# apache/auron

Hardware: AMD Instinct MI355X
Metric: tpcds_suite_seconds (lower is better)
Workload: dtype decimal64/fp64

## Files before the change

### auron_amd/column.py

```python
from __future__ import annotations

from typing import Iterable, List, Optional, Sequence

import torch

from . import dtypes
from .dtypes import DataType


class Column:
    __slots__ = ("dtype", "data", "validity", "offsets")

    def __init__(
        self,
        dtype: DataType,
        data: torch.Tensor,
        validity: Optional[torch.Tensor] = None,
        offsets: Optional[torch.Tensor] = None,
    ):
        self.dtype = dtype
        self.data = data
        self.validity = validity
        self.offsets = offsets
        if dtype.uses_offsets:
# ... 77 lines not shown
                    limbs.append(((lo - (1 << 64)) if lo >= (1 << 63) else lo,
                                  iv >> 64))
                data = torch.tensor(limbs, dtype=torch.int64) if limbs else \
                    torch.empty((0, 2), dtype=torch.int64)
            else:
                data = torch.tensor(tvals, dtype=dtype.torch_dtype)
            col = Column(dtype, data, validity, None)
        assert len(col) == n
        return col.to(device)

    def to_pylist(self) -> list:
        c = self.to("cpu")
        valid = None if c.validity is None else c.validity.tolist()
        if self.dtype.is_string:
            raw = bytes(c.data.numpy().tobytes())
            offs = c.offsets.tolist()
            out = []
            for i in range(len(c)):
                if valid is not None and not valid[i]:
                    out.append(None)
                else:
                    out.append(raw[offs[i]:offs[i + 1]].decode("utf-8", errors="replace"))
            return out
        if self.dtype.is_list:
            offs = c.offsets.tolist()
            flat = c.data.tolist()
            out = []
            for i in range(len(c)):
                if valid is not None and not valid[i]:
                    out.append(None)
                else:
                    out.append(flat[offs[i]:offs[i + 1]])
            return out
        if self.dtype.code == dtypes.DECIMAL128:
            s = 10 ** self.dtype.scale
            lo = c.data[:, 0].tolist()
            hi = c.data[:, 1].tolist()
            m64 = (1 << 64) - 1
            vals = [((h << 64) | (l & m64)) / s for l, h in zip(lo, hi)]
            if valid is None:
                return vals
            return [v if ok else None for v, ok in zip(vals, valid)]
        vals = c.data.tolist()
        if self.dtype.code == dtypes.DECIMAL64:
            s = 10 ** self.dtype.scale
            vals = [v / s for v in vals]
        if valid is None:
            return vals
        return [v if ok else None for v, ok in zip(vals, valid)]

    def gather(self, indices: torch.Tensor,
               may_have_negative: bool = False) -> "Column":
        idx = indices.to(self.device)
        neg = None
        if may_have_negative and idx.numel():
            neg = idx < 0
            idx = idx.clamp(min=0)
            if not bool(neg.any()) if idx.device.type != "cuda" else False:
                neg = None
        validity = None
        if self.validity is not None:
            validity = self.validity[idx]
        if neg is not None:
            if validity is None:
                validity = torch.ones(idx.shape[0], dtype=torch.bool, device=self.device)
            validity = validity & ~neg
        if self.dtype.uses_offsets:
            off = self.offsets.to(torch.int64)
            starts = off[idx]
            lens = off[idx + 1] - starts
            if neg is not None:
                lens = torch.where(neg, torch.zeros_like(lens), lens)
            new_off = torch.zeros(idx.shape[0] + 1, dtype=torch.int64, device=self.device)
            torch.cumsum(lens, 0, out=new_off[1:])
            total = int(new_off[-1].item())
            if total == 0:
                out_el = torch.empty(0, dtype=self.data.dtype, device=self.device)
            elif self.device.type == "cuda" and self.data.dtype == torch.uint8:
                from . import native

                out_el = torch.empty(total, dtype=torch.uint8, device=self.device)
                rc = native.lib().au_bytes_gather(
                    self.data.data_ptr(), starts.contiguous().data_ptr(),
                    new_off.data_ptr(), out_el.data_ptr(), idx.shape[0],
                    native.stream_ptr(self.device))
                native.check(rc, "au_bytes_gather")
            else:
                pos = torch.arange(total, dtype=torch.int64, device=self.device)
                row = torch.repeat_interleave(lens)
                el_idx = pos - new_off[:-1][row] + starts[row]
                out_el = self.data[el_idx]
            return Column(self.dtype, out_el, validity, new_off)
        data = self.data[idx]
        return Column(self.dtype, data, validity, None)

    def filter(self, mask: torch.Tensor) -> "Column":
        idx = torch.nonzero(mask, as_tuple=False).flatten()
        return self.gather(idx)

    def slice(self, start: int, length: int) -> "Column":
        idx = torch.arange(start, start + length, dtype=torch.int64, device=self.device)
        return self.gather(idx)

    @staticmethod
    def concat(cols: List["Column"]) -> "Column":
        assert cols
# ... 99 lines not shown
            t = torch.from_numpy(np_arr)
            if t.dtype != dt.torch_dtype:
                t = t.to(dt.torch_dtype)
            col = Column(dt, t, validity, None)
        return col.to(device)

    def to_arrow(self):
        import numpy as np
        import pyarrow as pa

        c = self.to("cpu")
        mask = None
        if c.validity is not None:
            mask = ~c.validity.numpy()
        if self.dtype.is_string:
            vals = c.to_pylist()
            return pa.array(vals, type=pa.string())
        if self.dtype.code == dtypes.DECIMAL64:
            from decimal import Decimal

            sc = self.dtype.scale
            vals = [None if (mask is not None and mask[i])
                    else Decimal(int(c.data[i].item())).scaleb(-sc)
                    for i in range(len(c))]
            p = max(self.dtype.precision, sc + 1, 1)
            return pa.array(vals, type=pa.decimal128(p, sc))
        if self.dtype.code == dtypes.DECIMAL128:
            from decimal import Context, Decimal

            wide = Context(prec=80)
            sc = self.dtype.scale
            lo = c.data[:, 0].numpy()
            hi = c.data[:, 1].numpy()
            vals = []
            for i in range(len(c)):
                if mask is not None and mask[i]:
                    vals.append(None)
                else:
                    v = (int(hi[i]) << 64) | (int(lo[i]) & ((1 << 64) - 1))
                    vals.append(Decimal(v).scaleb(-sc, context=wide))
            p = max(self.dtype.precision, sc + 1, 1)
            return pa.array(vals, type=pa.decimal128(min(p, 38), sc))
        np_arr = c.data.numpy()
        if self.dtype.code == dtypes.TIMESTAMP:
            return pa.array(np_arr, from_pandas=False, mask=mask).cast(
                pa.timestamp("us"))
        return pa.array(np_arr, from_pandas=False, mask=mask)

    def __repr__(self) -> str:
        return f"Column({self.dtype.name}, n={len(self)}, nulls={self.null_count}, dev={self.device})"



def compact_validity(v: Optional[torch.Tensor]) -> Optional[torch.Tensor]:
    if v is None or v.device.type == "cuda":
        return v
    return None if bool(v.all()) else v


def adjacent_equal(c: Column, nan_equal: bool = False) -> torch.Tensor:
    n = len(c)
    if n <= 1:
        return torch.zeros(0, dtype=torch.bool, device=c.device)
    a = c.gather(torch.arange(0, n - 1, dtype=torch.int64, device=c.device))
    b = c.gather(torch.arange(1, n, dtype=torch.int64, device=c.device))
    if c.dtype.is_string:
        from . import strings as S

        eq = S.compare(a, b, "==")
    else:
        eq = a.data == b.data
        if nan_equal and c.dtype.is_float:
            eq = eq | (torch.isnan(a.data) & torch.isnan(b.data))
    ones = torch.ones(n - 1, dtype=torch.bool, device=c.device)
    av = a.validity if a.validity is not None else ones
    bv = b.validity if b.validity is not None else ones
    return (eq & av & bv) | (~av & ~bv)


class RecordBatch:
    __slots__ = ("names", "columns", "_eval_memo")

    def __init__(self, names: List[str], columns: List[Column]):
        assert len(names) == len(columns)
        if columns:
            n = len(columns[0])
            for c in columns:
                assert len(c) == n, f"ragged batch: {[len(x) for x in columns]}"
        self.names = list(names)
        self.columns = list(columns)

    @property
    def num_rows(self) -> int:
        return len(self.columns[0]) if self.columns else 0

    @property
    def num_columns(self) -> int:
        return len(self.columns)

    @property
    def device(self) -> torch.device:
        return self.columns[0].device if self.columns else torch.device("cpu")

    def column(self, name: str) -> Column:
        return self.columns[self.names.index(name)]

    def to(self, device) -> "RecordBatch":
        return RecordBatch(self.names, [c.to(device) for c in self.columns])

    def gather(self, idx: torch.Tensor,
               may_have_negative: bool = False) -> "RecordBatch":
        if self.device.type == "cuda" and len(self.columns) > 1:
            fused = self._gather_fused(idx, may_have_negative)
            if fused is not None:
                return fused
        return RecordBatch(self.names,
                           [c.gather(idx, may_have_negative) for c in self.columns])

    def _gather_fused(self, idx: torch.Tensor, may_have_negative: bool):
        from . import native

        if not native.available():
            return None
        import numpy as np

        lib = native.lib()
        idx = idx.to(self.device).to(torch.int64).contiguous()
        n = int(idx.numel())
        out_cols: list = [None] * len(self.columns)
        descs = []
        keep = [idx]
        for ci, c in enumerate(self.columns):
            if c.dtype.uses_offsets:
                out_cols[ci] = c.gather(idx, may_have_negative)
                continue
            data = c.data if c.data.is_contiguous() else c.data.contiguous()
            keep.append(data)
            esize = data.element_size() * (2 if c.dtype.code == dtypes.DECIMAL128 else 1)
            shape = (n, 2) if c.dtype.code == dtypes.DECIMAL128 else (n,)
            dst = torch.empty(shape, dtype=data.dtype, device=self.device)
            want_valid = c.validity is not None or may_have_negative
            dv = torch.empty(n, dtype=torch.bool, device=self.device) \
                if want_valid else None
            sv = 0
            if c.validity is not None:
                v = c.validity if c.validity.is_contiguous() else c.validity.contiguous()
                keep.append(v)
                sv = v.data_ptr()
            descs.append((data.data_ptr(), sv, dst.data_ptr(),
                          dv.data_ptr() if dv is not None else 0, esize, 0))
            out_cols[ci] = Column(c.dtype, dst, dv)
        if descs and n:
            arr = np.array(descs, dtype=np.uint64).reshape(-1, 6)
            arr = np.ascontiguousarray(arr)
            for lo in range(0, len(descs), 24):
                sub = np.ascontiguousarray(arr[lo:lo + 24])
                rc = lib.au_multi_gather(idx.data_ptr(), n, sub.ctypes.data,
                                         sub.shape[0],
                                         native.stream_ptr(self.device))
                native.check(rc, "au_multi_gather")
        return RecordBatch(self.names, out_cols)

    def filter(self, mask: torch.Tensor) -> "RecordBatch":
        idx = torch.nonzero(mask, as_tuple=False).flatten()
        return self.gather(idx)

    def slice(self, start: int, length: int) -> "RecordBatch":
        return RecordBatch(self.names, [c.slice(start, length) for c in self.columns])

    def select(self, names: Iterable[str]) -> "RecordBatch":
        names = list(names)
        return RecordBatch(names, [self.column(n) for n in names])

    @staticmethod
    def concat(batches: List["RecordBatch"]) -> "RecordBatch":
        assert batches
        names = batches[0].names
        cols = [Column.concat([b.columns[i] for b in batches]) for i in range(len(names))]
        return RecordBatch(names, cols)

    @staticmethod
    def from_pydict(d: dict, types: dict, device="cpu") -> "RecordBatch":
        names = list(d.keys())
        cols = [Column.from_pylist(d[n], types[n], device) for n in names]
        return RecordBatch(names, cols)
# ... 31 lines not shown
```

### auron_amd/config.py

```python
from __future__ import annotations

import os
from dataclasses import dataclass
from typing import Any, Dict, Optional


@dataclass(frozen=True)
class ConfigOption:
    key: str
    default: Any
    typ: type
    doc: str = ""
    env: Optional[str] = None


_REGISTRY: Dict[str, ConfigOption] = {}


def _opt(key: str, default, typ, doc="", env=None) -> ConfigOption:
    o = ConfigOption(key, default, typ, doc, env)
    _REGISTRY[key] = o
    return o


# ... 64 lines not shown
                               env="AURON_SORT_EXTERNAL_WIDE_KEYS")
EXCHANGE_SAMPLE_ROWS = _opt("spark.auron.rangePartition.sampleRows", 4096, int,
                            "per-rank sample size for range-partition bounds")
SCAN_CACHE_BYTES = _opt("spark.auron.scan.cache.maxBytes", 0, int,
                        "per-query decoded-scan cache budget; 0 = auto "
                        "(15% of HBM on GPU, 4 GB on CPU)",
                        env="AURON_SCAN_CACHE_BYTES")
STREAM_BYTES = _opt("spark.auron.stream.minInputBytes", -1, int,
                    "estimated agg-input bytes above which operators "
                    "stream instead of materializing; -1 = auto (8% of "
                    "HBM on GPU, 1 GB on CPU), 0 = always stream",
                    env="AURON_STREAM_BYTES")
SCAN_HBM_CACHE = _opt("spark.auron.scan.hbmStagedCache.maxBytes", 0, int,
                      "staged raw-page bytes kept device-resident across "
                      "reads; 0 = auto (30% of HBM)",
                      env="AURON_SCAN_HBM_CACHE")
HBM_CACHE_RESERVE = _opt("spark.auron.scan.hbmStagedCache.reserveFraction",
                         0.25, float,
                         "free-HBM fraction the staged-bytes cache must "
                         "never consume (evicts itself under pressure)")
SCAN_DELTA_NATIVE = _opt("spark.auron.scan.deltaNative.enable", True, bool,
                         "decode DELTA_BINARY_PACKED pages and "
                         "DELTA_LENGTH_BYTE_ARRAY / DELTA_BYTE_ARRAY string "
                         "pages with the k_pq_delta_* kernels from a "
                         "host-built miniblock index, DELTA_BYTE_ARRAY "
                         "strings rebuilt by k_pq_dba_bytes (off: "
                         "DELTA_BINARY_PACKED is expanded to PLAIN by one "
                         "host job per page and DELTA_LENGTH_BYTE_ARRAY and "
                         "DELTA_BYTE_ARRAY columns take the pyarrow host "
                         "read)",
                         env="AURON_SCAN_DELTA_NATIVE")
SCAN_PREFETCH = _opt("spark.auron.scan.streamPrefetch", 2, int,
                     "files decoded ahead of the consumer on the "
                     "streaming scan path")
SCAN_IO_THREADS = _opt("spark.auron.scan.ioThreads", 8, int,
                       "host page-read/staging thread-pool size",
                       env="AURON_SCAN_IO_THREADS")
STREAM_PEEK_FACTOR = _opt("spark.auron.stream.peekBatches", 8, int,
                          "batch-size multiples buffered before the "
                          "chunked agg commits to streaming")
STREAM_JOIN_PROBE = _opt("spark.auron.stream.joinProbe.enable", True, bool,
                         "probe build-right joins batch-by-batch on the "
                         "streaming path (GPU only)",
                         env="AURON_STREAM_JOIN_PROBE")
JOIN_FUSED_PROBE = _opt("spark.auron.join.fusedProbe.enable", True, bool,
                        "probe hash joins with the fused kernels "
                        "(k_join_probe_count / k_join_probe_fill / "
                        "k_join_exists: probe hash computed in-kernel, one "
                        "chain walk, per-tile offsets, key descriptors passed "
                        "by value) for up to 8 key columns (off: murmur3 + "
                        "k_join_count + torch scan + k_join_fill, and "
                        "join_counts for semi/anti/existence joins)",
                        env="AURON_JOIN_FUSED_PROBE")
DECIMAL128_NATIVE_ARITH = _opt("spark.auron.decimal128.nativeArith.enable",
                               True, bool,
                               "run exact decimal128 + - * /, comparisons, "
                               "casts, abs and CheckOverflow on the "
                               "k_dec128_* kernels (off: the exact "
                               "host-integer reference path, also on GPU "
                               "batches)",
                               env="AURON_DECIMAL128_NATIVE_ARITH")
SPILL_DIR = _opt("spark.auron.spill.dir", "", str,
                 "directory for disk-tier spill files (empty = system tmp)",
                 env="AURON_SPILL_DIR")
MEM_BUDGET = _opt("spark.auron.memory.budgetBytes", 0, int,
                  "absolute memmgr budget override; 0 = memoryFraction "
                  "of device/host memory", env="AURON_MEM_BUDGET")


class AuronConf:
    def __init__(self, overrides: Optional[Dict[str, Any]] = None):
        self._values: Dict[str, Any] = {}
        if overrides:
            for k, v in overrides.items():
                self.set(k, v)

    def set(self, key: str, value) -> "AuronConf":
        if key not in _REGISTRY:
            raise KeyError(f"unknown config {key}; known: {sorted(_REGISTRY)}")
        self._values[key] = value
        return self

    def get(self, opt: ConfigOption):
        if opt.key in self._values:
            return self._values[opt.key]
        if opt.env and opt.env in os.environ:
            raw = os.environ[opt.env]
            if opt.typ is bool:
                return raw not in ("0", "false", "False")
            return opt.typ(raw)
        return opt.default

    @staticmethod
    def options() -> Dict[str, ConfigOption]:
        return dict(_REGISTRY)
```

### auron_amd/engine/executor.py

```python
from __future__ import annotations

import os
import time
from dataclasses import dataclass, field
from typing import Dict, List, Optional

import torch
import torch.distributed as dist

from .. import dtypes, ops
from ..column import Column, RecordBatch, adjacent_equal, compact_validity
from ..dtypes import DataType
from ..exchange import all_gather_batch, all_to_all
from ..exprs import AggFunc, Col
from ..plan import nodes as P
from ..config import AGG_STREAMING, BROADCAST_CACHE_BYTES, AuronConf
from .window import exec_window


@dataclass
class ExecContext:
    device: torch.device = torch.device("cpu")
    rank: int = 0
    world_size: int = 1
# ... 50 lines not shown
    return None if p is None else (p, 0)


def _decimal128_key_type(a, b):
    if dtypes.DECIMAL128 not in (a.code, b.code):
        return None
    if a.code == b.code and a.scale == b.scale:
        return None
    oa, ob = _decimal_key_operand(a), _decimal_key_operand(b)
    if oa is None or ob is None:
        return None
    (p1, s1), (p2, s2) = oa, ob
    s = max(s1, s2)
    digits = max(p1 - s1, p2 - s2)
    if s + digits > dtypes.MAX_DECIMAL_PRECISION:
        return None
    return dtypes.decimal128(s + digits, s)


def _normalize_join_keys(lkeys, rkeys):
    from ..exprs import _cast_col, _promote

    lo, ro = [], []
    for l, r in zip(lkeys, rkeys):
        common = _decimal128_key_type(l.dtype, r.dtype)
        if common is not None:
            l, r = _cast_col(l, common), _cast_col(r, common)
        elif (l.dtype.code == r.dtype.code == dtypes.DECIMAL128
              and l.dtype.scale != r.dtype.scale):
            l = _cast_col(l, dtypes.float64)
            r = _cast_col(r, dtypes.float64)
        elif l.dtype.code != r.dtype.code:
            l, r, _ = _promote(l, r)
        lo.append(l)
        ro.append(r)
    return lo, ro


class TaskCancelled(RuntimeError):
    """Raised inside execute() after Executor.cancel()."""


def _cast_for_range(c: Column) -> Column:
    if c.dtype.is_string:
        raise NotImplementedError("range partitioning on string keys")
    return c


def _concat(batches: List[RecordBatch]) -> RecordBatch:
    assert batches, "executor invariant violated: empty batch list"
    if len(batches) == 1:
        return batches[0]
    return RecordBatch.concat(batches)


def _empty_like(batch: RecordBatch) -> RecordBatch:
    idx = torch.empty(0, dtype=torch.int64, device=batch.device)
    return batch.gather(idx)



def _expr_sig(exprs) -> bytes:
    import hashlib

    from ..plan.serde import serialize_plan
    from ..plan import serde as _serde
    import msgpack as _mp

    return hashlib.sha1(_mp.packb([_serde._encode(e) for e in exprs],
                                  use_bin_type=True)).digest()


def _cacheable_build(plan) -> bool:
    if isinstance(plan, (P.MemoryScan, P.PyUdf, P.PyUdaf, P.Generate)):
        return False
    return all(_cacheable_build(c) for c in plan.children())


class Executor:
    def __init__(self, ctx: Optional[ExecContext] = None):
        self.ctx = ctx or ExecContext.from_dist()
        self._child_time = [0.0]
        import collections as _collections

        self._scan_cache: "_collections.OrderedDict" = _collections.OrderedDict()
        self._fused_progs: Dict[int, tuple] = {}
        self._scan_cache_bytes = 0
        self._metric_stack: List[list] = [[]]
        self.last_metric_tree: Optional[dict] = None
        import threading

        self._cancelled = threading.Event()
        self._io_pool = None

    def _scan_pool(self):
        if self._io_pool is None:
            from concurrent.futures import ThreadPoolExecutor

            from ..config import SCAN_IO_THREADS

            self._io_pool = ThreadPoolExecutor(
                max_workers=AuronConf().get(SCAN_IO_THREADS),
                thread_name_prefix="auron-io")
        return self._io_pool

    def cancel(self):
# ... 1137 lines not shown
            batches = itertools.chain(buf, rest)
        schema_batch: Optional[RecordBatch] = None
        limit = self.ctx.batch_rows
        acc: List[RecordBatch] = []
        acc_rows = 0
        merge_worthwhile = True
        holder = self.ctx.memmgr.register("agg-partial-state", acc)

        def flush_merge():
            nonlocal acc, acc_rows, merge_worthwhile, holder
            cur = holder.batches()
            merged = self._merge_states(node, _concat(cur)) if cur else None
            holder.release()
            if merged is not None:
                if merged.num_rows > 0.8 * acc_rows:
                    merge_worthwhile = False
                acc = [merged]
                acc_rows = merged.num_rows
            else:
                acc = []
                acc_rows = 0
            holder = self.ctx.memmgr.register("agg-partial-state", acc)

        for b in batches:
            if schema_batch is None:
                schema_batch = b.slice(0, 0)
            for lo in range(0, max(b.num_rows, 1), limit):
                chunk = b if b.num_rows <= limit else \
                    b.slice(lo, min(limit, b.num_rows - lo))
                with eval_scope(chunk):
                    out = self._hash_agg_body(node, chunk)
                cur = holder.batches()
                cur.extend(out)
                acc_rows += sum(x.num_rows for x in out)
                holder.refresh()
                if b.num_rows <= limit:
                    break
            if merge_worthwhile and acc_rows > 2 * limit:
                flush_merge()
        result = holder.batches()
        holder.release()
        if not result:
            assert schema_batch is not None, "child stream yielded no batches"
            with eval_scope(schema_batch):
                return self._hash_agg_body(node, schema_batch)
        return result

    def _merge_states(self, node: P.HashAgg, b: RecordBatch) -> RecordBatch:
        device = b.device
        key_cols = [Col(a.name).eval(b) for a in node.keys]
        if key_cols:
            gids, reps = ops.group_ids(key_cols)
            ngroups = int(reps.numel())
            out_keys = [c.gather(reps) for c in key_cols]
        else:
            gids = torch.zeros(b.num_rows, dtype=torch.int64, device=device)
            ngroups = 1 if b.num_rows else 0
            out_keys = []
        names = [a.name for a in node.keys]
        cols = list(out_keys)
        for i, agg in enumerate(node.aggs):
            s0 = b.column(f"__agg{i}_0")
            s1 = b.column(f"__agg{i}_1")
            merged_cnt, _ = ops.agg_scatter(gids, ngroups, s1, "sum")
            if agg.fn in ("count", "count_star"):
                cols.append(Column(dtypes.int64, merged_cnt))
                names.append(f"__agg{i}_0")
                cols.append(Column(dtypes.int64, merged_cnt))
                names.append(f"__agg{i}_1")
                continue
            comb = {"sum": "sum", "avg": "sum", "min": "min", "max": "max",
                    "first": "first", "first_ignores_null": "first"}[agg.fn]
            if comb == "first":
                acc_col, _ = self._agg_first(gids, ngroups, s0)
                cols.append(acc_col)
            elif comb == "sum" and s0.dtype.code == dtypes.DECIMAL128:
                data, cnt = self._sum128_scatter(gids, ngroups, s0)
                cols.append(Column(s0.dtype, data, compact_validity(cnt > 0)))
            elif comb == "sum" and self._decimal_sum_unsafe(s0, b.num_rows):
                data, cnt = self._sum_split_exact(gids, ngroups, s0)
                cols.append(Column(s0.dtype, data, cnt > 0))
            else:
                data, cnt = ops.agg_scatter(gids, ngroups, s0, comb)
                if isinstance(data, Column):
                    cols.append(data)
                else:
                    cols.append(Column(s0.dtype, data, compact_validity(cnt > 0)))
            names.append(f"__agg{i}_0")
            cols.append(Column(dtypes.int64, merged_cnt))
            names.append(f"__agg{i}_1")
        return RecordBatch(names, cols)

    def _hash_agg_body(self, node: P.HashAgg, b: RecordBatch) -> List[RecordBatch]:
        device = b.device
        n = b.num_rows
        if node.mode == "final":
            key_cols = [Col(a.name).eval(b) for a in node.keys]
        else:
            key_cols = [a.expr.eval(b) for a in node.keys]
        if node.keys:
            if node.mode == "partial" and self._partial_skip(key_cols, n):
                return [self._partial_passthrough(node, b, key_cols)]
            gids, reps = ops.group_ids(key_cols)
            ngroups = int(reps.numel())
            out_keys = [c.gather(reps) for c in key_cols]
        else:
            gids = torch.zeros(n, dtype=torch.int64, device=device)
            if n == 0 and node.mode in ("final", "complete") and self.ctx.rank != 0:
                ngroups = 0
            else:
                ngroups = 1
            out_keys = []
        names = [a.name for a in node.keys]
        cols = list(out_keys)
        fused: Dict[int, tuple] = {}
        if node.mode in ("partial", "complete") and ngroups > 0:
            fuse_items = []
            fuse_idx = []
            for i, agg in enumerate(node.aggs):
                if agg.fn in ("sum", "avg", "min", "max") and agg.expr is not None:
                    v = agg.expr.eval(b)
                    if v.dtype.code == dtypes.DECIMAL128:
                        continue
                    if agg.fn == "sum" and self._sum_needs_128(v.dtype):
                        continue
                    if agg.fn in ("sum", "avg") and self._decimal_sum_unsafe(v, n):
                        continue
                    fuse_items.append((v, agg.fn))
                    fuse_idx.append(i)
            if len(fuse_items) > 1:
                for i, res in zip(fuse_idx,
                                  ops.agg_scatter_multi(gids, ngroups, fuse_items)):
                    fused[i] = (fuse_items[fuse_idx.index(i)][0], res)
        for i, agg in enumerate(node.aggs):
            s0, s1 = f"__agg{i}_0", f"__agg{i}_1"
            if node.mode == "final":
                sv = b.column(s0)
                sc = b.column(s1)
                merged_cnt, _ = ops.agg_scatter(gids, ngroups, sc, "sum")
                if agg.fn in ("count", "count_star"):
                    cols.append(Column(dtypes.int64, merged_cnt))
                    names.append(agg.name)
                    continue
                comb = {"sum": "sum", "avg": "sum", "min": "min", "max": "max",
                        "first": "first", "first_ignores_null": "first"}[agg.fn]
                if comb == "first":
                    acc, cnt = self._agg_first(gids, ngroups, sv)
                elif comb == "sum" and sv.dtype.code == dtypes.DECIMAL128:
                    data, cnt = self._sum128_scatter(gids, ngroups, sv)
                    acc = Column(sv.dtype, data, compact_validity(cnt > 0))
                elif comb == "sum" and self._decimal_sum_unsafe(sv, n):
                    acc, cnt = self._sum_split_exact(gids, ngroups, sv)
                else:
                    acc, cnt = ops.agg_scatter(gids, ngroups, sv, comb)
                cols.append(self._finalize_agg(agg, sv.dtype, acc, merged_cnt,
                                                widen=False))
                names.append(agg.name)
            else:
# ... 352 lines not shown
                                      existence_col=node.existence_col,
                                      residual=node.residual)
                return self._exec_SortMergeJoin(smj)
        lkeys = [k.eval(left) for k in node.left_keys]
        rkeys = [k.eval(right) for k in node.right_keys]
        lkeys, rkeys = _normalize_join_keys(lkeys, rkeys)
        how = node.how
        device = self.ctx.device

        table = None
        if cache_entry is not None and node.build_side == "right":
            sig = _expr_sig(node.right_keys)
            table = cache_entry["tables"].get(sig)
            if table is None:
                table = ops.join_build(rkeys)
                if table is not None:
                    cache_entry["tables"][sig] = table
                    self.ctx.broadcast_cache_bytes += table.nbytes

        if node.residual is not None:
            bi, pi, _ = ops.hash_join(rkeys, lkeys,
                                      emit_unmatched_probe=False,
                                      need_build_matched=False,
                                      table=table)
            return self._finish_join_pairs(left, right, pi, bi, how,
                                           node.residual, node.existence_col)

        if how in ("semi", "anti", "existence"):
            matched = ops.join_exists(rkeys, lkeys, table=table)
            if how == "semi":
                return [left.filter(matched)]
            if how == "anti":
                return [left.filter(~matched)]
            exists = Column(dtypes.bool_, matched)
            return [RecordBatch(left.names + [node.existence_col], left.columns + [exists])]

        preserved = {"inner": set(), "left": {"left"}, "right": {"right"},
                     "full": {"left", "right"}}[how]
        build_side = node.build_side
        probe_side = "left" if build_side == "right" else "right"
        build_keys, probe_keys = (rkeys, lkeys) if build_side == "right" else (lkeys, rkeys)
        bi, pi, bmatched = ops.hash_join(
            build_keys, probe_keys,
            emit_unmatched_probe=(probe_side in preserved),
            need_build_matched=(build_side in preserved),
            table=table if build_side == "right" else None,
        )
        if build_side in preserved and bmatched is not None:
            un = torch.nonzero(~bmatched, as_tuple=False).flatten()
            if un.numel():
                bi = torch.cat([bi, un])
                pi = torch.cat([pi, torch.full((un.numel(),), -1, dtype=torch.int64, device=bi.device)])
        li, ri = (pi, bi) if build_side == "right" else (bi, pi)
        out_left = left.gather(li, may_have_negative=True)
        out_right = right.gather(ri, may_have_negative=True)
        return [RecordBatch(out_left.names + out_right.names,
                            out_left.columns + out_right.columns)]

    def _finish_join_pairs(self, left: RecordBatch, right: RecordBatch,
                           li: torch.Tensor, ri: torch.Tensor, how: str,
                           residual, existence_col: str) -> List[RecordBatch]:
        device = self.ctx.device
        if residual is not None and li.numel():
            pair = RecordBatch(left.names + right.names,
                               left.gather(li).columns + right.gather(ri).columns)
            m = residual.eval(pair)
            keep = m.data
            if m.validity is not None:
                keep = keep & m.validity
            li, ri = li[keep], ri[keep]
        nl, nr = left.num_rows, right.num_rows
        if how in ("semi", "anti", "existence"):
            lmatched = torch.zeros(nl, dtype=torch.bool, device=device)
            if li.numel():
                lmatched[li] = True
            if how == "semi":
                return [left.filter(lmatched)]
            if how == "anti":
                return [left.filter(~lmatched)]
            return [RecordBatch(left.names + [existence_col],
                                left.columns + [Column(dtypes.bool_, lmatched)])]
        preserved = {"inner": set(), "left": {"left"}, "right": {"right"},
                     "full": {"left", "right"}}[how]
        if "left" in preserved:
            lm = torch.zeros(nl, dtype=torch.bool, device=device)
            if li.numel():
                lm[li] = True
            un = torch.nonzero(~lm, as_tuple=False).flatten()
            if un.numel():
                li = torch.cat([li, un])
                ri = torch.cat([ri, torch.full((un.numel(),), -1,
                                               dtype=torch.int64, device=device)])
        if "right" in preserved:
            rm = torch.zeros(nr, dtype=torch.bool, device=device)
            matched_r = ri[ri >= 0]
            if matched_r.numel():
                rm[matched_r] = True
            un = torch.nonzero(~rm, as_tuple=False).flatten()
            if un.numel():
                ri = torch.cat([ri, un])
                li = torch.cat([li, torch.full((un.numel(),), -1,
                                               dtype=torch.int64, device=device)])
        out_left = left.gather(li, may_have_negative=True)
        out_right = right.gather(ri, may_have_negative=True)
        return [RecordBatch(out_left.names + out_right.names,
                            out_left.columns + out_right.columns)]

    def _exec_PyUdaf(self, node: P.PyUdaf) -> List[RecordBatch]:
        b = _concat(self.execute(node.child))
        device = b.device
        n = b.num_rows
        key_cols = [a.expr.eval(b) for a in node.keys]
        if key_cols:
            gids, reps = ops.group_ids(key_cols)
            ngroups = int(reps.numel())
            out_keys = [c.gather(reps) for c in key_cols]
        else:
            gids = torch.zeros(n, dtype=torch.int64, device=device)
            ngroups = 1
            out_keys = []
        in_vals = [e.eval(b).to("cpu").to_pylist() for e in node.inputs]
        gl = gids.to("cpu").tolist()
        buckets: List[List[int]] = [[] for _ in range(ngroups)]
        for i, g in enumerate(gl):
            buckets[g].append(i)
        results = []
        for rows in buckets:
            args = [[vals[i] for i in rows] for vals in in_vals]
            results.append(node.fn(*args))
        names = [a.name for a in node.keys]
        cols = list(out_keys)
        for j, (cname, cdt) in enumerate(node.out_schema):
            vals = [r[j] if isinstance(r, tuple) else r for r in results]
            cols.append(Column.from_pylist(vals, cdt, str(device)))
            names.append(cname)
        return [RecordBatch(names, cols)]

    def _exec_Window(self, node: P.Window) -> List[RecordBatch]:
        return exec_window(self, node, _concat(self.execute(node.child)))
```

### auron_amd/native/__init__.py

```python
from __future__ import annotations

import ctypes
import os
from typing import List, Optional, Tuple

import numpy as np
import torch

_LIB_NAME = "libauron_hip.so"
_here = os.path.dirname(os.path.abspath(__file__))
LIB_PATH = os.path.join(_here, _LIB_NAME)

_lib = None
_load_error: Optional[str] = None


class AuronNativeMissing(RuntimeError):
    pass


def _try_load():
    global _lib, _load_error
    if _lib is not None or _load_error is not None:
        return
    if not os.path.exists(LIB_PATH):
        _load_error = f"{LIB_PATH} not built (run python -m auron_amd.native.build)"
        return
    try:
        lib = ctypes.CDLL(LIB_PATH)
    except OSError as e:
        _load_error = str(e)
        return
    c = ctypes.c_void_p
    i32 = ctypes.c_int32
    i64 = ctypes.c_int64
    lib.au_abi_version.restype = ctypes.c_int
    lib.au_murmur3.argtypes = [c, ctypes.c_int, i64, i32, c, c]
    lib.au_group_ids.argtypes = [c, ctypes.c_int, i64, c, i64, c, c, c, c, c, c]
    lib.au_join_build.argtypes = [i64, c, i64, c, c, c]
    lib.au_join_count.argtypes = [c, c, ctypes.c_int, i64, c, i64, c, c, c, c]
    lib.au_join_fill.argtypes = [c, c, ctypes.c_int, i64, c, i64, c, c, c, c, c, c, ctypes.c_int, c]
    lib.au_join_probe_tile.argtypes = []
    lib.au_join_probe_tile.restype = i64
    lib.au_join_probe_max_keys.argtypes = []
    lib.au_join_probe_max_keys.restype = ctypes.c_int
    lib.au_join_probe_count.argtypes = [c, ctypes.c_int, i64, c, i64, c, i32,
                                        ctypes.c_int, c, c, c, c, c]
    lib.au_join_probe_fill.argtypes = [c, ctypes.c_int, i64, c, c, c, c,
                                       ctypes.c_int, c, c, c]
    lib.au_join_exists.argtypes = [c, ctypes.c_int, i64, c, i64, c, i32, c, c]
    for f in ("au_join_probe_count", "au_join_probe_fill", "au_join_exists"):
        getattr(lib, f).restype = ctypes.c_int
    lib.au_pmod.argtypes = [c, i64, i32, c, c]
    lib.au_bytes_gather.argtypes = [c, c, c, c, i64, c]
    lib.au_multi_gather.argtypes = [c, i64, c, ctypes.c_int, c]
    lib.au_multi_gather.restype = ctypes.c_int
    lib.au_agg_scatter.argtypes = [c, i64, c, c, ctypes.c_int, ctypes.c_int,
                                   ctypes.c_int, c, c, i64, c]
    lib.au_agg_count.argtypes = [c, i64, c, c, c]
    lib.au_agg_multi.argtypes = [c, i64, c, ctypes.c_int, c]
    for f in ("au_agg_scatter", "au_agg_count", "au_agg_multi"):
        getattr(lib, f).restype = ctypes.c_int
    lib.au_pq_rle1.argtypes = [c, ctypes.c_int, c, c, c]
    lib.au_rle1_expand.argtypes = [c, i64, c, c, c]
    lib.au_rle1_expand.restype = ctypes.c_int
    lib.au_host_rle1_parse.argtypes = [c, i64, i64, i64, i64, c, i64]
    lib.au_host_rle1_parse.restype = i64
    lib.au_host_plainba_parse.argtypes = [c, i64, i64, c, c, i64]
    lib.au_host_plainba_parse.restype = i64
    lib.au_host_delta_unpack.argtypes = [c, i64, i64, i64, ctypes.c_int, c]
    lib.au_host_delta_unpack.restype = i64
    lib.au_host_delta_index.argtypes = [c, i64, i64, i64, i64, i64, i64, c, c,
                                        i64]
    lib.au_host_delta_index.restype = i64
    lib.au_pq_delta_sums.argtypes = [c, i64, c, c, c]
    lib.au_pq_delta_scan.argtypes = [c, i64, c]
    lib.au_pq_delta_emit.argtypes = [c, i64, c, i64, c, c, c, ctypes.c_int, c]
    for f in ("au_pq_delta_sums", "au_pq_delta_scan", "au_pq_delta_emit"):
        getattr(lib, f).restype = ctypes.c_int
    lib.au_host_dba_decode.argtypes = [c, i64, c, c, c, c, i64, c, i64]
    lib.au_host_dba_decode.restype = i64
    lib.au_pq_dba_tile.argtypes = []
    lib.au_pq_dba_tile.restype = i64
    lib.au_pq_dba_bytes.argtypes = [c, c, c, c, i64, i64, c, c, c]
    lib.au_pq_dba_bytes.restype = ctypes.c_int
    lib.au_pq_rle_idx.argtypes = [c, ctypes.c_int, c, c, c, c]
    lib.au_pq_scatter.argtypes = [c, ctypes.c_int, c, c, c, c, ctypes.c_int, i64, c]
    lib.au_pq_copy_plain.argtypes = [c, ctypes.c_int, c, c, ctypes.c_int, i64, c]
    for f in ("au_pq_rle1", "au_pq_rle_idx", "au_pq_scatter", "au_pq_copy_plain"):
        getattr(lib, f).restype = ctypes.c_int
    lib.au_expr_exec.argtypes = [c, ctypes.c_int, c, ctypes.c_int, c,
                                 ctypes.c_int, ctypes.c_int, i64, c]
    lib.au_expr_exec.restype = ctypes.c_int
    lib.au_part_hist.argtypes = [c, i64, i32, c, c]
    lib.au_part_scatter.argtypes = [c, i64, c, c, c, c]
    lib.au_range_bucket_str.argtypes = [c, c, i64, c, c, i32, ctypes.c_int, c, c]
    lib.au_range_bucket_i128.argtypes = [c, i64, c, i32, ctypes.c_int, c, c]
    for f in ("au_range_bucket_str", "au_range_bucket_i128"):
        getattr(lib, f).restype = ctypes.c_int
    f64 = ctypes.c_double
    lib.au_window_range_bounds_i64.argtypes = [c, c, c, i64, i64, i64,
                                               ctypes.c_int, c, c, c]
    lib.au_window_range_bounds_f64.argtypes = [c, c, c, i64, f64, f64,
                                               ctypes.c_int, c, c, c]
    lib.au_window_frame_minmax_i64.argtypes = [c, i64, c, i64, c, c, i64,
                                               ctypes.c_int, c, c]
    lib.au_window_frame_minmax_f64.argtypes = [c, i64, c, i64, c, c, i64,
                                               ctypes.c_int, c, c]
    lib.au_window_pyramid_size.argtypes = [i64]
# ... 111 lines not shown
```

### auron_amd/native/csrc/kernels.hip

```cpp

#include <hip/hip_runtime.h>
#include <stdint.h>

#define AU_EXPORT extern "C" __attribute__((visibility("default")))

enum AuDType : int32_t {
  AU_BOOL = 0,
  AU_INT8 = 1,
  AU_INT16 = 2,
  AU_INT32 = 3,
  AU_INT64 = 4,
  AU_FLOAT32 = 5,
  AU_FLOAT64 = 6,
  AU_DATE32 = 7,
  AU_STRING = 8,
  AU_DECIMAL64 = 9,
  AU_LIST = 10,
  AU_TIMESTAMP = 11,
  AU_DECIMAL128 = 12,
};

struct AuColDesc {
  const void* data;
  const int64_t* offsets;
// ... 741 lines not shown
struct MgCol {
  const void* src;
  const uint8_t* src_valid;
  void* dst;
  uint8_t* dst_valid;
  int64_t esize;
  int64_t pad;
};

struct MgParams { MgCol cols[MG_MAX_COLS]; };

__global__ void __launch_bounds__(256) k_multi_gather(
    const int64_t* __restrict__ idx, int64_t n, MgParams p, int ncols) {
  int64_t chunks_per_col = (n + 255) / 256;
  for (int64_t b = blockIdx.x; b < chunks_per_col * ncols; b += gridDim.x) {
    int c = (int)(b / chunks_per_col);
    int64_t row = (b % chunks_per_col) * 256 + threadIdx.x;
    if (row >= n) continue;
    const MgCol col = p.cols[c];
    int64_t i = idx[row];
    bool ok = i >= 0;
    int64_t src_i = ok ? i : 0;
    bool v = ok && (!col.src_valid || col.src_valid[src_i]);
    if (col.dst_valid) col.dst_valid[row] = v;
    switch (col.esize) {
      case 1: ((uint8_t*)col.dst)[row] = ok ? ((const uint8_t*)col.src)[src_i] : 0; break;
      case 2: ((uint16_t*)col.dst)[row] = ok ? ((const uint16_t*)col.src)[src_i] : 0; break;
      case 4: ((uint32_t*)col.dst)[row] = ok ? ((const uint32_t*)col.src)[src_i] : 0; break;
      case 8: ((uint64_t*)col.dst)[row] = ok ? ((const uint64_t*)col.src)[src_i] : 0; break;
      case 16: {
        ulonglong2 z; z.x = 0; z.y = 0;
        ((ulonglong2*)col.dst)[row] = ok ? ((const ulonglong2*)col.src)[src_i] : z;
        break;
      }
      default: break;
    }
  }
}

AU_EXPORT int au_multi_gather(const void* idx, int64_t n,
                              const void* host_cols, int ncols,
                              void* stream) {
  if (n <= 0 || ncols <= 0) return 0;
  if (ncols > MG_MAX_COLS) return 1002;
  MgParams p{};
  const MgCol* hc = (const MgCol*)host_cols;
  for (int i = 0; i < ncols; i++) p.cols[i] = hc[i];
  int64_t chunks = ((n + 255) / 256) * ncols;
  int64_t g = chunks > 4096 ? 4096 : chunks;
  hipLaunchKernelGGL(k_multi_gather, dim3((uint32_t)g), dim3(256), 0,
                     (hipStream_t)stream, (const int64_t*)idx, n, p, ncols);
  return (int)hipGetLastError();
}
```

Baseline: 2.987.

## Gather string columns with batched native size/scan/fill kernels

Adds HIP kernels that gather up to 8 string columns per launch. One kernel sums tile byte sizes, one scans them, and one writes offsets, validity and bytes in-kernel. This replaces the per-column torch indexing, cumsum and sync path, and it is wired into column gather, batch fused gather and group-key gathers. Joins now pass may_have_negative only for sides that can actually receive -1 indices. The change risks extra launches for small batches and still needs one host read of the byte totals per batch.

```diff
diff --git a/auron_amd/column.py b/auron_amd/column.py
--- a/auron_amd/column.py
+++ b/auron_amd/column.py
@@ -153,6 +153,8 @@
     def gather(self, indices: torch.Tensor,
                may_have_negative: bool = False) -> "Column":
         idx = indices.to(self.device)
+        if _native_string_col(self) and _native_strings_enabled():
+            return gather_strings_native([self], idx, may_have_negative)[0]
         neg = None
         if may_have_negative and idx.numel():
             neg = idx < 0
@@ -358,6 +360,88 @@
 
 
 
+STR_GATHER_MAX_COLS = 8
+
+
+def _native_strings_enabled() -> bool:
+    from .config import GATHER_NATIVE_STRINGS, AuronConf
+
+    return bool(AuronConf().get(GATHER_NATIVE_STRINGS))
+
+
+def _native_string_col(c: Column) -> bool:
+    return (c.dtype.is_string and c.data.dtype == torch.uint8
+            and c.device.type == "cuda")
+
+
+def gather_strings_native(cols: List[Column], idx: torch.Tensor,
+                          may_have_negative: bool = False) -> List[Column]:
+    if not cols:
+        return []
+    import numpy as np
+
+    from . import native
+
+    lib = native.lib()
+    device = cols[0].device
+    idx = idx.to(device).to(torch.int64).contiguous()
+    n = int(idx.numel())
+    if n == 0:
+        return [Column(c.dtype, torch.empty(0, dtype=torch.uint8, device=device),
+                       None if c.validity is None else c.validity[idx],
+                       torch.zeros(1, dtype=torch.int64, device=device))
+                for c in cols]
+    nc = len(cols)
+    n_tiles = (n + 1023) // 1024
+    stream = native.stream_ptr(device)
+    tile_sums = torch.empty(nc * n_tiles, dtype=torch.int64, device=device)
+    totals = torch.empty(nc, dtype=torch.int64, device=device)
+    descs = np.zeros((nc, 6), dtype=np.uint64)
+    keep = []
+    new_offs, valids = [], []
+    for k, c in enumerate(cols):
+        for part in (c.offsets, c.validity):
+            if part is not None and part.device != device:
+                raise ValueError(f"column buffers on {device} and "
+                                 f"{part.device}: move the whole Column")
+        data, off = c.data.contiguous(), c.offsets.contiguous()
+        keep += [data, off]
+        descs[k, 0] = data.data_ptr()
+        descs[k, 1] = off.data_ptr()
+        if c.validity is not None:
+            v = c.validity.contiguous()
+            keep.append(v)
+            descs[k, 2] = v.data_ptr()
+        new_offs.append(torch.empty(n + 1, dtype=torch.int64, device=device))
+        descs[k, 4] = new_offs[k].data_ptr()
+        valids.append(torch.empty(n, dtype=torch.bool, device=device)
+                      if c.validity is not None or may_have_negative else None)
+        if valids[k] is not None:
+            descs[k, 5] = valids[k].data_ptr()
+    chunks = [(lo, min(lo + STR_GATHER_MAX_COLS, nc))
+              for lo in range(0, nc, STR_GATHER_MAX_COLS)]
+    for lo, hi in chunks:
+        sub = np.ascontiguousarray(descs[lo:hi])
+        rc = lib.au_str_gather_sizes(
+            idx.data_ptr(), n, sub.ctypes.data, hi - lo,
+            tile_sums.data_ptr() + lo * n_tiles * 8,
+            totals.data_ptr() + lo * 8, stream)
+        native.check(rc, "au_str_gather_sizes")
+    sizes = totals.tolist()
+    outs = [torch.empty(t, dtype=torch.uint8, device=device) for t in sizes]
+    for k, o in enumerate(outs):
+        descs[k, 3] = o.data_ptr()
+    for lo, hi in chunks:
+        sub = np.ascontiguousarray(descs[lo:hi])
+        rc = lib.au_str_gather_fill(
+            idx.data_ptr(), n, sub.ctypes.data, hi - lo,
+            tile_sums.data_ptr() + lo * n_tiles * 8,
+            totals.data_ptr() + lo * 8, stream)
+        native.check(rc, "au_str_gather_fill")
+    return [Column(c.dtype, o, v, off)
+            for c, o, v, off in zip(cols, outs, valids, new_offs)]
+
+
 def compact_validity(v: Optional[torch.Tensor]) -> Optional[torch.Tensor]:
     if v is None or v.device.type == "cuda":
         return v
@@ -436,7 +520,14 @@
         out_cols: list = [None] * len(self.columns)
         descs = []
         keep = [idx]
+        str_at = [ci for ci, c in enumerate(self.columns)
+                  if _native_string_col(c)] if _native_strings_enabled() else []
+        for ci, sc in zip(str_at, gather_strings_native(
+                [self.columns[ci] for ci in str_at], idx, may_have_negative)):
+            out_cols[ci] = sc
         for ci, c in enumerate(self.columns):
+            if out_cols[ci] is not None:
+                continue
             if c.dtype.uses_offsets:
                 out_cols[ci] = c.gather(idx, may_have_negative)
                 continue
diff --git a/auron_amd/config.py b/auron_amd/config.py
--- a/auron_amd/config.py
+++ b/auron_amd/config.py
@@ -140,6 +140,16 @@
                         "k_join_count + torch scan + k_join_fill, and "
                         "join_counts for semi/anti/existence joins)",
                         env="AURON_JOIN_FUSED_PROBE")
+GATHER_NATIVE_STRINGS = _opt("spark.auron.gather.nativeStrings.enable", True,
+                             bool,
+                             "gather the string columns of a GPU batch with "
+                             "the batch kernels (k_sg_sizes / k_sg_scan / "
+                             "k_sg_fill: output offsets, validity and bytes "
+                             "written in-kernel, up to 8 columns per launch, "
+                             "one host read of the byte totals per batch) "
+                             "(off: per column, torch index / cumsum glue, "
+                             "one sync and k_bytes_gather)",
+                             env="AURON_GATHER_NATIVE_STRINGS")
 DECIMAL128_NATIVE_ARITH = _opt("spark.auron.decimal128.nativeArith.enable",
                                True, bool,
                                "run exact decimal128 + - * /, comparisons, "
diff --git a/auron_amd/engine/executor.py b/auron_amd/engine/executor.py
--- a/auron_amd/engine/executor.py
+++ b/auron_amd/engine/executor.py
@@ -126,6 +126,11 @@
     if len(batches) == 1:
         return batches[0]
     return RecordBatch.concat(batches)
+
+
+def _gather_keys(key_cols: List[Column], reps: torch.Tensor) -> List[Column]:
+    names = [f"k{i}" for i in range(len(key_cols))]
+    return RecordBatch(names, key_cols).gather(reps).columns
 
 
 def _empty_like(batch: RecordBatch) -> RecordBatch:
@@ -1369,7 +1374,7 @@
         if key_cols:
             gids, reps = ops.group_ids(key_cols)
             ngroups = int(reps.numel())
-            out_keys = [c.gather(reps) for c in key_cols]
+            out_keys = _gather_keys(key_cols, reps)
         else:
             gids = torch.zeros(b.num_rows, dtype=torch.int64, device=device)
             ngroups = 1 if b.num_rows else 0
@@ -1420,7 +1425,7 @@
                 return [self._partial_passthrough(node, b, key_cols)]
             gids, reps = ops.group_ids(key_cols)
             ngroups = int(reps.numel())
-            out_keys = [c.gather(reps) for c in key_cols]
+            out_keys = _gather_keys(key_cols, reps)
         else:
             gids = torch.zeros(n, dtype=torch.int64, device=device)
             if n == 0 and node.mode in ("final", "complete") and self.ctx.rank != 0:
@@ -1879,8 +1884,8 @@
                 bi = torch.cat([bi, un])
                 pi = torch.cat([pi, torch.full((un.numel(),), -1, dtype=torch.int64, device=bi.device)])
         li, ri = (pi, bi) if build_side == "right" else (bi, pi)
-        out_left = left.gather(li, may_have_negative=True)
-        out_right = right.gather(ri, may_have_negative=True)
+        out_left = left.gather(li, may_have_negative="right" in preserved)
+        out_right = right.gather(ri, may_have_negative="left" in preserved)
         return [RecordBatch(out_left.names + out_right.names,
                             out_left.columns + out_right.columns)]
 
@@ -1928,8 +1933,8 @@
                 ri = torch.cat([ri, un])
                 li = torch.cat([li, torch.full((un.numel(),), -1,
                                                dtype=torch.int64, device=device)])
-        out_left = left.gather(li, may_have_negative=True)
-        out_right = right.gather(ri, may_have_negative=True)
+        out_left = left.gather(li, may_have_negative="right" in preserved)
+        out_right = right.gather(ri, may_have_negative="left" in preserved)
         return [RecordBatch(out_left.names + out_right.names,
                             out_left.columns + out_right.columns)]
 
@@ -1941,7 +1946,7 @@
         if key_cols:
             gids, reps = ops.group_ids(key_cols)
             ngroups = int(reps.numel())
-            out_keys = [c.gather(reps) for c in key_cols]
+            out_keys = _gather_keys(key_cols, reps)
         else:
             gids = torch.zeros(n, dtype=torch.int64, device=device)
             ngroups = 1
diff --git a/auron_amd/native/__init__.py b/auron_amd/native/__init__.py
--- a/auron_amd/native/__init__.py
+++ b/auron_amd/native/__init__.py
@@ -55,6 +55,14 @@
     lib.au_bytes_gather.argtypes = [c, c, c, c, i64, c]
     lib.au_multi_gather.argtypes = [c, i64, c, ctypes.c_int, c]
     lib.au_multi_gather.restype = ctypes.c_int
+    lib.au_str_gather_tile.argtypes = []
+    lib.au_str_gather_tile.restype = i64
+    lib.au_str_gather_max_cols.argtypes = []
+    lib.au_str_gather_max_cols.restype = ctypes.c_int
+    lib.au_str_gather_sizes.argtypes = [c, i64, c, ctypes.c_int, c, c, c]
+    lib.au_str_gather_fill.argtypes = [c, i64, c, ctypes.c_int, c, c, c]
+    for f in ("au_str_gather_sizes", "au_str_gather_fill"):
+        getattr(lib, f).restype = ctypes.c_int
     lib.au_agg_scatter.argtypes = [c, i64, c, c, ctypes.c_int, ctypes.c_int,
                                    ctypes.c_int, c, c, i64, c]
     lib.au_agg_count.argtypes = [c, i64, c, c, c]
diff --git a/auron_amd/native/csrc/kernels.hip b/auron_amd/native/csrc/kernels.hip
--- a/auron_amd/native/csrc/kernels.hip
+++ b/auron_amd/native/csrc/kernels.hip
@@ -817,3 +817,202 @@
                      (hipStream_t)stream, (const int64_t*)idx, n, p, ncols);
   return (int)hipGetLastError();
 }
+
+#define SG_MAX_COLS 8
+
+struct SgCol {
+  const uint8_t* src;
+  const int64_t* src_off;
+  const uint8_t* src_valid;
+  uint8_t* dst;
+  int64_t* dst_off;
+  uint8_t* dst_valid;
+};
+
+struct SgParams { SgCol cols[SG_MAX_COLS]; };
+
+__global__ void __launch_bounds__(JP_BLOCK) k_sg_sizes(
+    const int64_t* __restrict__ idx, int64_t n, int64_t n_tiles, SgParams p,
+    int ncols, int64_t* __restrict__ tile_sums) {
+  __shared__ int64_t wsum[JP_BLOCK / 64];
+  const int tid = threadIdx.x;
+  for (int64_t w = blockIdx.x; w < n_tiles * ncols; w += gridDim.x) {
+    const int64_t* __restrict__ off = p.cols[w / n_tiles].src_off;
+    const int64_t base = (w % n_tiles) * JP_TILE;
+    int64_t acc = 0;
+#pragma unroll
+    for (int s = 0; s < JP_SLABS; s++) {
+      const int64_t row = base + s * JP_BLOCK + tid;
+      if (row >= n) continue;
+      const int64_t i = idx[row];
+      if (i >= 0) acc += off[i + 1] - off[i];
+    }
+    for (int d = 32; d > 0; d >>= 1) acc += __shfl_down(acc, d, 64);
+    if ((tid & 63) == 0) wsum[tid >> 6] = acc;
+    __syncthreads();
+    if (tid == 0) {
+      int64_t sum = 0;
+      for (int k = 0; k < JP_BLOCK / 64; k++) sum += wsum[k];
+      tile_sums[w] = sum;
+    }
+    __syncthreads();
+  }
+}
+
+__global__ void __launch_bounds__(JP_BLOCK) k_sg_scan(
+    int64_t* __restrict__ tile_sums, int64_t n_tiles,
+    int64_t* __restrict__ totals) {
+  __shared__ int64_t wtot[2][JP_BLOCK / 64];
+  const int tid = threadIdx.x;
+  const int lane = tid & 63, wave = tid >> 6;
+  int64_t* __restrict__ sums = tile_sums + (int64_t)blockIdx.x * n_tiles;
+  int64_t running = 0;
+  int buf = 0;
+  for (int64_t t0 = 0; t0 < n_tiles; t0 += JP_BLOCK, buf ^= 1) {
+    const int64_t t = t0 + tid;
+    const int64_t v = t < n_tiles ? sums[t] : 0;
+    int64_t incl = v;
+    for (int d = 1; d < 64; d <<= 1) {
+      int64_t up = __shfl_up(incl, d, 64);
+      if (lane >= d) incl += up;
+    }
+    if (lane == 63) wtot[buf][wave] = incl;
+    __syncthreads();
+    int64_t before = 0, total = 0;
+    for (int k = 0; k < JP_BLOCK / 64; k++) {
+      const int64_t x = wtot[buf][k];
+      if (k < wave) before += x;
+      total += x;
+    }
+    if (t < n_tiles) sums[t] = running + before + incl - v;
+    running += total;
+  }
+  if (tid == 0) totals[blockIdx.x] = running;
+}
+
+__device__ __forceinline__ void sg_copy_row(const uint8_t* __restrict__ from,
+                                            uint8_t* __restrict__ to,
+                                            int64_t len) {
+  if (len >= 8) {
+    uint64_t x;
+    for (int64_t j = 0; j + 8 < len; j += 8) {
+      __builtin_memcpy(&x, from + j, 8);
+      __builtin_memcpy(to + j, &x, 8);
+    }
+    __builtin_memcpy(&x, from + len - 8, 8);
+    __builtin_memcpy(to + len - 8, &x, 8);
+    return;
+  }
+  if (len & 4) {
+    uint32_t x;
+    __builtin_memcpy(&x, from, 4);
+    __builtin_memcpy(to, &x, 4);
+  }
+  if (len & 2) {
+    uint16_t x;
+    __builtin_memcpy(&x, from + (len & 4), 2);
+    __builtin_memcpy(to + (len & 4), &x, 2);
+  }
+  if (len & 1) to[len & 6] = from[len & 6];
+}
+
+__global__ void __launch_bounds__(JP_BLOCK) k_sg_fill(
+    const int64_t* __restrict__ idx, int64_t n, int64_t n_tiles, SgParams p,
+    int ncols, const int64_t* __restrict__ tile_bases,
+    const int64_t* __restrict__ totals) {
+  __shared__ int64_t wtot[2][JP_SLABS][JP_BLOCK / 64];
+  const int tid = threadIdx.x;
+  const int lane = tid & 63, wave = tid >> 6;
+  int buf = 0;
+  for (int64_t w = blockIdx.x; w < n_tiles * ncols; w += gridDim.x, buf ^= 1) {
+    const int c = (int)(w / n_tiles);
+    const SgCol col = p.cols[c];
+    const int64_t base = (w % n_tiles) * JP_TILE;
+    int64_t i[JP_SLABS], s0[JP_SLABS], len[JP_SLABS], incl[JP_SLABS];
+#pragma unroll
+    for (int s = 0; s < JP_SLABS; s++) {
+      const int64_t row = base + s * JP_BLOCK + tid;
+      i[s] = row < n ? idx[row] : -1;
+    }
+#pragma unroll
+    for (int s = 0; s < JP_SLABS; s++) {
+      s0[s] = 0;
+      len[s] = 0;
+      if (i[s] >= 0) {
+        s0[s] = col.src_off[i[s]];
+        len[s] = col.src_off[i[s] + 1] - s0[s];
+      }
+    }
+#pragma unroll
+    for (int s = 0; s < JP_SLABS; s++) {
+      incl[s] = len[s];
+      for (int d = 1; d < 64; d <<= 1) {
+        int64_t up = __shfl_up(incl[s], d, 64);
+        if (lane >= d) incl[s] += up;
+      }
+      if (lane == 63) wtot[buf][s][wave] = incl[s];
+    }
+    __syncthreads();
+    int64_t running = tile_bases[w];
+#pragma unroll
+    for (int s = 0; s < JP_SLABS; s++) {
+      int64_t before = 0, total = 0;
+      for (int k = 0; k < JP_BLOCK / 64; k++) {
+        const int64_t x = wtot[buf][s][k];
+        if (k < wave) before += x;
+        total += x;
+      }
+      const int64_t d0 = running + before + incl[s] - len[s];
+      running += total;
+      const int64_t row = base + s * JP_BLOCK + tid;
+      if (row >= n) continue;
+      col.dst_off[row] = d0;
+      if (row == n - 1) col.dst_off[n] = totals[c];
+      if (col.dst_valid)
+        col.dst_valid[row] =
+            i[s] >= 0 && (!col.src_valid || col.src_valid[i[s]]);
+      sg_copy_row(col.src + s0[s], col.dst + d0, len[s]);
+    }
+  }
+}
+
+AU_EXPORT int64_t au_str_gather_tile() { return JP_TILE; }
+AU_EXPORT int au_str_gather_max_cols() { return SG_MAX_COLS; }
+
+static inline int sg_grid(int64_t items) {
+  return (int)(items > 4096 ? 4096 : items);
+}
+
+AU_EXPORT int au_str_gather_sizes(const int64_t* idx, int64_t n,
+                                  const void* host_cols, int ncols,
+                                  int64_t* tile_sums, int64_t* totals,
+                                  void* stream) {
+  if (n <= 0 || ncols <= 0) return 0;
+  if (ncols > SG_MAX_COLS) return 1002;
+  SgParams p{};
+  const SgCol* hc = (const SgCol*)host_cols;
+  for (int i = 0; i < ncols; i++) p.cols[i] = hc[i];
+  const int64_t n_tiles = (n + JP_TILE - 1) / JP_TILE;
+  hipLaunchKernelGGL(k_sg_sizes, dim3(sg_grid(n_tiles * ncols)), dim3(JP_BLOCK),
+                     0, (hipStream_t)stream, idx, n, n_tiles, p, ncols,
+                     tile_sums);
+  hipLaunchKernelGGL(k_sg_scan, dim3(ncols), dim3(JP_BLOCK), 0,
+                     (hipStream_t)stream, tile_sums, n_tiles, totals);
+  return (int)hipGetLastError();
+}
+
+AU_EXPORT int au_str_gather_fill(const int64_t* idx, int64_t n,
+                                 const void* host_cols, int ncols,
+                                 const int64_t* tile_bases,
+                                 const int64_t* totals, void* stream) {
+  if (n <= 0 || ncols <= 0) return 0;
+  if (ncols > SG_MAX_COLS) return 1002;
+  SgParams p{};
+  const SgCol* hc = (const SgCol*)host_cols;
+  for (int i = 0; i < ncols; i++) p.cols[i] = hc[i];
+  const int64_t n_tiles = (n + JP_TILE - 1) / JP_TILE;
+  hipLaunchKernelGGL(k_sg_fill, dim3(sg_grid(n_tiles * ncols)), dim3(JP_BLOCK),
+                     0, (hipStream_t)stream, idx, n, n_tiles, p, ncols,
+                     tile_bases, totals);
+  return (int)hipGetLastError();
+}
diff --git a/profiles/measure_batch_gather.py b/profiles/measure_batch_gather.py
--- /dev/null
+++ b/profiles/measure_batch_gather.py
@@ -0,0 +1,109 @@
+import argparse
+import json
+import os
+import statistics
+import sys
+import time
+
+import numpy as np
+import torch
+
+sys.path.insert(0, os.path.join(os.path.dirname(os.path.abspath(__file__)), ".."))
+from auron_amd import dtypes, native
+from auron_amd.column import Column, RecordBatch
+
+DEV = "cuda:0"
+ENV = "AURON_GATHER_NATIVE_STRINGS"
+
+
+def _str_col(rng, n, lo, hi):
+    lens = np.full(n, lo, dtype=np.int64) if lo == hi else rng.integers(lo, hi + 1, n)
+    offs = np.zeros(n + 1, dtype=np.int64)
+    np.cumsum(lens, out=offs[1:])
+    data = rng.integers(32, 127, int(offs[-1]), dtype=np.uint8)
+    return Column(dtypes.string, torch.from_numpy(data).to(DEV), None,
+                  torch.from_numpy(offs).to(DEV))
+
+
+def _customer_like(rng, n):
+    cols = [_str_col(rng, n, 16, 16), _str_col(rng, n, 8, 20), _str_col(rng, n, 8, 20)]
+    cols += [Column(dtypes.int64, torch.from_numpy(rng.integers(0, 1 << 40, n)).to(DEV))
+             for _ in range(2)]
+    return RecordBatch(["id", "first", "last", "sk", "addr"], cols)
+
+
+def _timed(fn, warm, reps):
+    out = {}
+    dev = {"0": [], "1": []}
+    host = {"0": [], "1": []}
+    for s in ("0", "1"):
+        os.environ[ENV] = s
+        for _ in range(warm):
+            out[s] = fn()
+    torch.cuda.synchronize()
+    for _ in range(reps):
+        for s in ("0", "1"):
+            os.environ[ENV] = s
+            e0 = torch.cuda.Event(enable_timing=True)
+            e1 = torch.cuda.Event(enable_timing=True)
+            t0 = time.perf_counter()
+            e0.record()
+            out[s] = fn()
+            e1.record()
+            torch.cuda.synchronize()
+            host[s].append((time.perf_counter() - t0) * 1e3)
+            dev[s].append(e0.elapsed_time(e1))
+    os.environ.pop(ENV, None)
+
+    def stat(v):
+        return {"median": round(statistics.median(v), 4), "min": round(min(v), 4),
+                "max": round(max(v), 4)}
+
+    return out["0"], out["1"], \
+        {"device_ms": stat(dev["0"]), "host_ms": stat(host["0"])}, \
+        {"device_ms": stat(dev["1"]), "host_ms": stat(host["1"])}
+
+
+def _same(a, b):
+    for x, y in zip(a.columns, b.columns):
+        for p, q in ((x.data, y.data), (x.offsets, y.offsets), (x.validity, y.validity)):
+            if (p is None) != (q is None) or (p is not None and not torch.equal(p, q)):
+                return False
+    return True
+
+
+def main():
+    ap = argparse.ArgumentParser()
+    ap.add_argument("--reps", type=int, default=20)
+    args = ap.parse_args()
+    assert torch.cuda.is_available(), "needs a GPU"
+    native.require()
+    rng = np.random.default_rng(0)
+
+    def case(name, batch, idx, flag=False):
+        off, on, t_off, t_on = _timed(lambda: batch.gather(idx, flag), 3, args.reps)
+        str_bytes = sum(int(c.data.numel()) for c in on.columns if c.offsets is not None)
+        print(json.dumps({
+            "case": name, "src_rows": batch.num_rows, "out_rows": int(idx.numel()),
+            "out_string_bytes": str_bytes, "same_result": _same(off, on),
+            "legacy": t_off, "native": t_on,
+            "speedup_device": round(t_off["device_ms"]["median"]
+                                    / t_on["device_ms"]["median"], 3),
+            "speedup_host": round(t_off["host_ms"]["median"]
+                                  / t_on["host_ms"]["median"], 3)}), flush=True)
+
+    cust = _customer_like(rng, 500_000)
+    big = torch.from_numpy(rng.integers(0, 500_000, 4_000_000)).to(DEV)
+    case("(a) customer join: 4M random rows of 500k", cust, big)
+    case("(b) small batch: 20k random rows of 500k", cust, big[:20_000].contiguous())
+    wide = _customer_like(rng, 8_000_000)
+    sel = torch.nonzero(torch.from_numpy(rng.random(8_000_000) < 0.5)).flatten().to(DEV)
+    case("(c) filter: monotone 50% of 8M rows", wide, sel)
+    del wide, sel
+    neg = big.clone()
+    neg[torch.from_numpy(rng.random(4_000_000) < 0.3).to(DEV)] = -1
+    case("(d) outer join: (a) with 30% -1, may_have_negative", cust, neg, True)
+
+
+if __name__ == "__main__":
+    main()
```

Result: faster. 2.606 (median of 4 runs) (-12.8%).
